# PKU-EPIC/GAPartNet

Measured on AMD Instinct MI355X. Metric: point-clouds/sec (20k pts, train step), higher is better.
Workload: dtype f32

## Files before the change

gapartnet_amd/_C.py:

```python
import ctypes
import os
import subprocess

_HERE = os.path.dirname(os.path.abspath(__file__))
SO_PATH = os.path.join(_HERE, "libgpn_hip.so")
CSRC = os.path.join(_HERE, "csrc")

_lib = None

_SIZE_T_FUNCS = (
    "gpn_voxelize_ws_bytes", "gpn_voxelize_scenes_ws_bytes", "gpn_rulebook_subm3_ws_bytes", "gpn_rulebook_down_ws_bytes",
    "gpn_rulebook_down_lists_ws_bytes", "gpn_rulebook_level_counts_ws_bytes", "gpn_spconv_fwd_ws_bytes", "gpn_spconv_fwd_w_ws_bytes", "gpn_net_ws_bytes", "gpn_linear_bwd_ws_bytes", "gpn_ball_query_grid_ws_bytes", "gpn_point_losses_ws_bytes", "gpn_rulebook_tile_order_ws_bytes", "gpn_bn_ws_bytes", "gpn_spconv_wgrad_ws_bytes", "gpn_ccl_ws_bytes", "gpn_nms_ws_bytes", "gpn_pn2_furthest_point_sampling_ws_bytes", "gpn_pose_fit_ws_bytes", "gpn_proposals_revoxelize_ws_bytes", "gpn_proposals_postprocess_ws_bytes", "gpn_backbone_prepare_arena_bytes", "gpn_scene_prepare_ws_bytes",
    "gpn_view_fps_ws_bytes", "gpn_net_forward_bf16_ws_bytes", "gpn_scene_maps_ws_bytes", "gpn_boxes_draw_ws_bytes",
    "gpn_pointmlp_wgrad_ws_bytes", "gpn_cloud_nearest_ws_bytes", "gpn_proposals_from_masks_ws_bytes",
    "gpn_render_ws_bytes", "gpn_frame_select_ws_bytes", "gpn_ground_mask_resize_ws_bytes", "gpn_ground_knn_ws_bytes",
    "gpn_cloud_grid_sample_ws_bytes",
)


class GpnError(RuntimeError):
    pass


def build(jobs: int = 8) -> str:
# ... 6 lines not shown
    if _lib is None:
        if not os.path.exists(SO_PATH):
            raise GpnError(
                f"{SO_PATH} is missing: the HIP extension has not been built. Run "
                "`python -c 'import __graft_entry__ as g; g.build()'` (needs hipcc). There is no CPU fallback.")
        import torch
        _lib = ctypes.CDLL(SO_PATH)
        _lib.gpn_last_error.restype = ctypes.c_char_p
        _lib.gpn_entry_point_name.restype = ctypes.c_char_p
        for name in _SIZE_T_FUNCS:
            getattr(_lib, name).restype = ctypes.c_size_t
        vp, i64t, i32t, f32t, st = ctypes.c_void_p, ctypes.c_int64, ctypes.c_int, ctypes.c_float, ctypes.c_size_t
        _lib.gpn_spconv_fwd_w.argtypes = [vp, vp, i32t, i32t, i32t, i32t, vp, i64t, vp, vp, st, vp]
        _lib.gpn_spconv_wgrad.argtypes = [vp, vp, vp, vp, vp, i32t, i64t, i32t, i32t, i32t, vp, vp, st, vp]
        _lib.gpn_bn_fwd_train.argtypes = [vp, vp, vp, vp, i64t, i32t, f32t, f32t, i32t, vp, vp, vp, vp, vp, vp, st, vp]
        _lib.gpn_bn_fwd_eval.argtypes = [vp, vp, vp, vp, vp, vp, i64t, i32t, i32t, vp, vp]
        _lib.gpn_bn_bwd.argtypes = [vp, vp, vp, vp, vp, vp, i64t, i32t, i32t, i32t, vp, vp, vp, vp, vp, st, vp]
        _lib.gpn_gather_rows.argtypes = [vp, vp, i64t, i32t, vp, vp]
        _lib.gpn_scatter_rows_csr.argtypes = [vp, vp, vp, i64t, i32t, vp, vp]
        _lib.gpn_spconv_tiles_min_tiles.argtypes = [i64t]
        _lib.gpn_spconv_tiles_min_tiles.restype = i64t
        _lib.gpn_spconv_direct_split.argtypes = [i64t, i64t]
        _lib.gpn_spconv_msplit.argtypes = [i32t, i32t, i32t]
    return _lib


def check(rc: int, what: str = ""):
    if rc != 0:
        msg = lib().gpn_last_error().decode("utf-8", "replace")
        raise GpnError(f"{what or 'gpn call'} failed (code {rc}): {msg}")


def ptr(t):
    if t is None:
        return ctypes.c_void_p(0)
    return ctypes.c_void_p(t.data_ptr())


def i64(v):
    return ctypes.c_int64(int(v))


def i32(v):
    return ctypes.c_int(int(v))


# ... 15 lines not shown
```

gapartnet_amd/csrc/gpn_core.hip:

```cpp
#include <cstdarg>
#include <algorithm>
#include <mutex>
#include <vector>

#include "gpn_common.h"

namespace {
thread_local char g_err[512] = "";

struct ProfRec {
  hipEvent_t a, b;
  int64_t tag;
};
struct ProfLive {
  const int64_t* rows_dev;
  int64_t bound;
  double flops, bytes;
};
struct ProfSlot {
  std::vector<ProfRec> recs;
  std::vector<ProfLive> live;
  double flops = 0, bytes = 0;
  int64_t launches = 0;
};
std::mutex g_prof_mu;
bool g_prof_on = false;
ProfSlot g_prof[GPN_K_COUNT];

const char* kEntryPoints[] = {
    "gpn_voxelize", "gpn_voxelize_ws_bytes", "gpn_rulebook_subm3", "gpn_rulebook_subm3_ws_bytes",
    "gpn_rulebook_down", "gpn_rulebook_down_ws_bytes", "gpn_rulebook_down_lists",
    "gpn_rulebook_down_lists_ws_bytes", "gpn_rulebook_level_counts", "gpn_rulebook_identity", "gpn_rulebook_level_counts_ws_bytes", "gpn_voxelize_ex", "gpn_voxelize_scenes", "gpn_voxelize_scenes_sorted", "gpn_voxelize_scenes_ws_bytes", "gpn_spconv_pack_weights", "gpn_spconv_fwd", "gpn_spconv_fwd_ws_bytes", "gpn_spconv_fwd_route", "gpn_spconv_fwd_ordered", "gpn_rulebook_tile_order_ws_bytes", "gpn_rulebook_tile_order", "gpn_spconv_tiles_min_tiles", "gpn_spconv_direct_split", "gpn_spconv_msplit", "gpn_spconv_fwd_w", "gpn_spconv_fwd_w_ws_bytes", "gpn_spconv_wgrad",
    "gpn_spconv_wgrad_ws_bytes", "gpn_gather_rows", "gpn_scatter_rows_csr", "gpn_bn_ws_bytes", "gpn_bn_fwd_train", "gpn_bn_fwd_eval", "gpn_bn_bwd", "gpn_net_ws_bytes", "gpn_net_bn_fusion", "gpn_net_wgrad_group", "gpn_net_forward", "gpn_linear_supported", "gpn_linear_fwd", "gpn_linear_bwd_ws_bytes", "gpn_linear_bwd", "gpn_net_backward", "gpn_net_forward_pair", "gpn_net_backward_pair", "gpn_point_losses_ws_bytes", "gpn_point_losses_fwd", "gpn_point_losses_fwd_metrics", "gpn_point_losses_bwd", "gpn_score_loss", "gpn_npcs_loss_fwd", "gpn_npcs_loss_bwd", "gpn_ball_query", "gpn_ball_query_grid_ws_bytes", "gpn_ball_query_grid", "gpn_ccl",
    "gpn_ccl_ws_bytes", "gpn_segmented_reduce", "gpn_segmented_maxpool_fwd", "gpn_segmented_maxpool_bwd",
    "gpn_instance_iou", "gpn_nms", "gpn_nms_ws_bytes", "gpn_pn2_ball_query", "gpn_pn2_group_points",
    "gpn_pn2_group_points_grad", "gpn_pn2_gather_points", "gpn_pn2_gather_points_grad",
    "gpn_pn2_furthest_point_sampling", "gpn_pn2_furthest_point_sampling_ws_bytes",
    "gpn_pn2_furthest_point_sampling_ws", "gpn_pn2_three_nn", "gpn_pn2_knn", "gpn_pn2_three_interpolate",
    "gpn_pn2_three_interpolate_grad", "gpn_proposals_max_proposals", "gpn_proposals_build_ws_bytes", "gpn_proposals_build", "gpn_proposals_voxel_mean",
    "gpn_proposals_voxel_mean_bwd", "gpn_proposals_revoxelize_ws_bytes", "gpn_proposals_revoxelize", "gpn_proposals_postprocess_ws_bytes", "gpn_proposals_postprocess", "gpn_proposals_postprocess_lds_proposals", "gpn_backbone_prepare_desc_words", "gpn_backbone_prepare_arena_bytes", "gpn_backbone_prepare", "gpn_scene_prepare_max_instances", "gpn_scene_prepare_ws_bytes", "gpn_scene_prepare", "gpn_pose_fit_ws_bytes", "gpn_pose_fit", "gpn_copy_many", "gpn_adam_blocks", "gpn_adam_step", "gpn_adam_step_gated", "gpn_prof_enable", "gpn_prof_bracket_overhead_us", "gpn_prof_reset", "gpn_prof_get", "gpn_prof_get_launches",
    "gpn_rulebook_subm3_dev", "gpn_rulebook_down_dev_ws_bytes", "gpn_rulebook_down_dev", "gpn_rulebook_down_lists_dev", "gpn_rulebook_identity_dev", "gpn_gather_rows_dev", "gpn_scatter_rows_csr_dev", "gpn_proposals_voxel_mean_dev", "gpn_proposals_targets_dev", "gpn_linear_fwd_dev", "gpn_linear_bwd_dev", "gpn_segmented_maxpool_fwd_dev", "gpn_segmented_maxpool_bwd_dev", "gpn_instance_iou_dev", "gpn_score_loss_dev", "gpn_npcs_loss_fwd_dev", "gpn_npcs_loss_bwd_dev",
    "gpn_view_max_instance_ids", "gpn_view_backproject", "gpn_view_fps_ws_bytes", "gpn_view_fps", "gpn_view_finish",
    "gpn_spconv_pack_weights_bf16", "gpn_spconv_fwd_bf16", "gpn_rows_to_bf16", "gpn_bn_act_bf16", "gpn_net_forward_bf16_ws_bytes",
    "gpn_net_forward_bf16",
    "gpn_scene_maps_ws_bytes", "gpn_scene_maps", "gpn_points_winner", "gpn_points_paint", "gpn_boxes_draw_ws_bytes", "gpn_boxes_draw",
    "gpn_pointmlp_supported", "gpn_pointmlp_fwd", "gpn_pointmlp_wgrad_ws_bytes", "gpn_pointmlp_wgrad",
    "gpn_cloud_pack", "gpn_cloud_finish", "gpn_cloud_nearest_ws_bytes", "gpn_cloud_nearest",
    "gpn_mask_pack", "gpn_proposals_from_masks_ws_bytes", "gpn_proposals_from_masks",
    "gpn_frame_backproject", "gpn_frame_select_ws_bytes", "gpn_frame_select",
    "gpn_cloud_grid_sample_ws_bytes", "gpn_cloud_grid_sample",
    "gpn_joint_sample", "gpn_cpd_rigid", "gpn_joint_from_rigid",
    "gpn_pose_gt_fit", "gpn_box_iou_3d", "gpn_pose_pair_errors",
    "gpn_render_max_links", "gpn_render_ws_bytes", "gpn_render_setup", "gpn_render_raster", "gpn_render_annotate",
    "gpn_render_max_lights", "gpn_render_shade",
    "gpn_ground_mask_resize_ws_bytes", "gpn_ground_mask_resize", "gpn_ground_mask_pool", "gpn_ground_bank_norms",
    "gpn_ground_knn_ws_bytes", "gpn_ground_knn",
// ... 135 lines not shown
```

gapartnet_amd/csrc/net.hip:

```cpp
#include <unistd.h>

#include <cstdlib>

#include <algorithm>
#include <atomic>
#include <condition_variable>
#include <mutex>
#include <string>
#include <thread>
#include <vector>

#include "gpn_common.h"
#include "spconv_pack.h"

namespace {

constexpr int kThreads = 256;

std::atomic<int> g_bn_fusion{1};

struct ConcatPtrs {
  const float4* a;
  const float4* b;
  float4* dst;
};
__global__ __launch_bounds__(kThreads) void concat_kernel(ConcatPtrs pa, ConcatPtrs pb, int64_t rows, int ca4, int cb4,
                                                          const int64_t* __restrict__ rows_dev) {
  rows = gpn::live_rows(rows_dev, rows);
  const ConcatPtrs& p = blockIdx.y ? pb : pa;
  const float4* __restrict__ a = p.a;
  const float4* __restrict__ b = p.b;
  float4* __restrict__ dst = p.dst;
  const int c4 = ca4 + cb4;
  const int64_t total = rows * c4;
  for (int64_t i = (int64_t)blockIdx.x * kThreads + threadIdx.x; i < total; i += (int64_t)gridDim.x * kThreads) {
    const int64_t r = i / c4;
    const int c = (int)(i - r * c4);
    dst[i] = c < ca4 ? a[r * ca4 + c] : b[r * cb4 + (c - ca4)];
  }
}

struct SplitPtrs {
// ... 50 lines not shown
  const PackDesc d = batch.d[blockIdx.y];
  const int64_t total = (int64_t)d.K * d.cin_w * d.cout_w;
  for (int64_t t = (int64_t)blockIdx.x * kThreads + threadIdx.x; t < total; t += (int64_t)gridDim.x * kThreads)
    d.packed[t] = gpn::packed_weight_element(d.W, d.K, d.cin_w, d.cout_w, d.flags, t);
}

inline int grid_for(int64_t total) {
  int64_t g = gpn::cdiv(total, kThreads);
  return (int)(g < 1 ? 1 : (g > 4096 ? 4096 : g));
}

inline size_t slot_bytes(const gpn_net_slot_t& s) { return (size_t)s.rows * s.channels * sizeof(float); }
inline gpn::DevRows dev_rows(const gpn_net_slot_t& s) { return gpn::DevRows{s.rows_dev, s.rows_plan}; }
inline int64_t plan_of(const gpn_net_slot_t& s) { return gpn::plan_rows(s.rows, dev_rows(s)); }

constexpr size_t kWgradBatchBytes = (size_t)96 << 20;

struct Need {
  size_t tmp = 0;
  size_t op = 0;
  size_t wgrad = 0;
  size_t packed = 0;
  size_t stats = 0;
};

Need workspace_need(const gpn_net_op_t* ops, int n_ops, const gpn_net_slot_t* slots, const gpn_net_rulebook_t* rbs,
                    const gpn_net_conv_t* convs) {
  Need n;
  size_t wgrad_sum = 0;
  for (int i = 0; i < n_ops; ++i) {
    const gpn_net_op_t& op = ops[i];
    const gpn_net_slot_t& s0 = slots[op.src0];
    if (op.kind == GPN_NET_CONV) {
      const gpn_net_rulebook_t& rb = rbs[op.rulebook];
      const gpn_net_conv_t& cv = convs[op.param];
      size_t w = gpn_spconv_fwd_ws_bytes(rb.K, rb.n_dst, cv.cin, cv.cout);
      size_t wt = gpn_spconv_fwd_ws_bytes(rb.K, rb.n_src, cv.cout, cv.cin);
      n.op = std::max(n.op, std::max(w, wt));
      const size_t wg = gpn_spconv_wgrad_ws_bytes(rb.K, cv.cin, cv.cout, rb.n_dst);
      n.wgrad = std::max(n.wgrad, wg);
      wgrad_sum += wg;
      n.packed += gpn::align_up((size_t)rb.K * cv.cin * cv.cout * sizeof(float));
      n.tmp = std::max(n.tmp, slot_bytes(s0));
    } else if (op.kind == GPN_NET_BN) {
      n.op = std::max(n.op, gpn_bn_ws_bytes(s0.rows, s0.channels));
      n.stats += gpn::stat_slab_bytes(s0.channels);
      if (op.src1 >= 0) n.tmp = std::max(n.tmp, slot_bytes(slots[op.src1]));
    }
  }
  n.tmp = gpn::align_up(n.tmp);
  n.op = gpn::align_up(n.op);
  n.wgrad = gpn::align_up(std::max(n.wgrad, std::min(wgrad_sum, kWgradBatchBytes)));
  return n;
}

int pack_program(const gpn_net_op_t* ops, int n_ops, const gpn_net_rulebook_t* rbs, const gpn_net_conv_t* convs,
                 bool transposed, char* area, std::vector<const float*>& packed_of, hipStream_t stream) {
  packed_of.assign(n_ops, nullptr);
  PackBatch batch;
  int fill = 0;
  int64_t max_total = 0;
  size_t off = 0;
  auto flush = [&]() -> int {
    if (fill == 0) return GPN_OK;
    int gx = (int)std::min<int64_t>(gpn::cdiv(max_total, kThreads), 256);
    hipLaunchKernelGGL(pack_many_kernel, dim3(gx, fill), dim3(kThreads), 0, stream, batch);
    hipError_t e = hipGetLastError();
    if (e != hipSuccess) {
      gpn::set_error("gpn_net: weight packing launch failed: %s", hipGetErrorString(e));
      return GPN_ERR_HIP;
    }
    fill = 0;
    max_total = 0;
    return GPN_OK;
  };
// ... 79 lines not shown
  return GPN_OK;
}

}

extern "C" int gpn_net_bn_fusion(int on) {
  return on < 0 ? g_bn_fusion.load(std::memory_order_relaxed) : g_bn_fusion.exchange(on ? 1 : 0, std::memory_order_relaxed);
}

namespace {
std::atomic<int>& wgrad_group_setting();
}
extern "C" int gpn_net_wgrad_group(int layers) {
  std::atomic<int>& g = wgrad_group_setting();
  if (layers < 1) return g.load(std::memory_order_relaxed);
  return g.exchange(layers > gpn::kWgradSets ? gpn::kWgradSets : layers, std::memory_order_relaxed);
}

extern "C" size_t gpn_net_ws_bytes(const gpn_net_op_t* ops, int n_ops, const gpn_net_slot_t* slots, int n_slots,
                                   const gpn_net_rulebook_t* rulebooks, const gpn_net_conv_t* convs) {
  (void)n_slots;
  if (!ops || !slots) return 0;
  const Need n = workspace_need(ops, n_ops, slots, rulebooks, convs);
  return n.tmp + n.op + n.wgrad + n.packed + n.stats;
}

namespace {

struct NetSet {
  gpn_net_slot_t* slots;
  const gpn_net_conv_t* convs;
  const gpn_net_bn_t* bns;
};

int net_forward_impl(const char* who, const gpn_net_op_t* ops, int n_ops, const NetSet* nets, int n_nets, int n_slots,
                     const gpn_net_rulebook_t* rbs, int n_rbs, int n_convs, int n_bns, int mode, void* ws, size_t ws_bytes,
                     hipStream_t stream) {
  const int training = mode == 1 ? 1 : 0;
  const bool inference = mode == GPN_NET_INFERENCE;
  if (mode != 0 && mode != 1 && mode != GPN_NET_INFERENCE) {
    gpn::set_error("%s: training must be 0, 1 or GPN_NET_INFERENCE", who);
    return GPN_ERR_ARG;
  }
  int rc = GPN_OK;
  for (int t = 0; t < n_nets; ++t) {
    rc = check_program(who, ops, n_ops, nets[t].slots, n_slots, rbs, n_rbs, nets[t].convs, n_convs, nets[t].bns, n_bns);
    if (rc) return rc;
// ... 181 lines not shown
                          (hipStream_t)stream_);
}

namespace {

std::atomic<int> g_wgrad_group{4};
std::atomic<int>& wgrad_group_setting() { return g_wgrad_group; }

constexpr int64_t g_wgrad_group_rows = 16384;

struct WgradJob {
  const float* in;
  const float* dout;
  const int32_t *pair_src, *pair_dst, *tile_off;
  int K;
  int64_t n_dst;
  gpn::DevRows rows;
  int cin, cout;
  float* dW;
  hipEvent_t after;
  const float* in2;
  const float* dout2;
  float* dW2;
};

class WgradWorker {
 public:
  void begin(int dev, hipStream_t side, void* ws, size_t ws_bytes, size_t max_jobs) {
    ensure_thread();
    jobs_.resize(max_jobs);
    dev_ = dev, side_ = side, ws_ = ws, ws_bytes_ = ws_bytes;
    published_.store(0, std::memory_order_relaxed);
    closed_.store(false, std::memory_order_relaxed);
    finished_.store(false, std::memory_order_relaxed);
    rc_ = GPN_OK;
    {
      std::lock_guard<std::mutex> lk(mu_);
      active_ = true;
    }
    cv_.notify_one();
  }
  void push(const WgradJob& j) {
    const size_t i = published_.load(std::memory_order_relaxed);
    jobs_[i] = j;
    published_.store(i + 1, std::memory_order_release);
  }
  int finish(std::string& err) {
    closed_.store(true, std::memory_order_release);
    while (!finished_.load(std::memory_order_acquire)) std::this_thread::yield();
    err = err_;
    return rc_;
  }

 private:
  void ensure_thread() {
    const pid_t pid = getpid();
    if (started_ && pid_ == pid) return;
    started_ = true;
    pid_ = pid;
    std::thread([this] { run(); }).detach();
  }
  void run() {
    for (;;) {
      {
        std::unique_lock<std::mutex> lk(mu_);
        cv_.wait(lk, [this] { return active_; });
        active_ = false;
      }
      (void)hipSetDevice(dev_);
      size_t done = 0;
      gpn::WgradReduceJob pending[gpn::kWgradReduceJobs];
      int n_pending = 0;
      size_t used = 0;
      const size_t room = std::min(ws_bytes_, kWgradBatchBytes);
      auto fail = [this](int rc) {
        if (rc_ == GPN_OK) {
          rc_ = rc;
          err_ = gpn_last_error();
        }
      };
      auto flush = [&] {
        if (n_pending && rc_ == GPN_OK) {
          const int rc = gpn::wgrad_reduce_many(pending, n_pending, side_);
          if (rc != GPN_OK) fail(rc);
        }
        n_pending = 0;
        used = 0;
      };
      WgradJob group[gpn::kWgradSets];
      int n_group = 0, group_sets = 0;
      auto same_shape = [](const WgradJob& a, const WgradJob& b) {
        return a.K == b.K && a.n_dst == b.n_dst && a.cin == b.cin && a.cout == b.cout && a.rows.dev == b.rows.dev;
      };
      auto launch_group = [&]() -> int {
        if (!n_group) return GPN_OK;
        const WgradJob& j0 = group[0];
        const int n = n_group, n_sets = group_sets;
        n_group = 0, group_sets = 0;
        if (hipStreamWaitEvent(side_, group[n - 1].after, 0) != hipSuccess) {
          gpn::set_error("gpn_net_backward: hipStreamWaitEvent failed on the weight-gradient stream");
          return GPN_ERR_HIP;
        }
        const size_t elems = (size_t)j0.K * j0.cin * j0.cout;
        if (j0.n_dst == 0) {
          for (int g = 0; g < n; ++g) {
            GPN_CHECK_HIP(hipMemsetAsync(group[g].dW, 0, sizeof(float) * elems, side_));
            if (group[g].dW2) GPN_CHECK_HIP(hipMemsetAsync(group[g].dW2, 0, sizeof(float) * elems, side_));
          }
          return GPN_OK;
        }
        const int S = gpn::wgrad_slices(j0.K, j0.cin, j0.cout, gpn::plan_rows(j0.n_dst, j0.rows));
        const size_t bytes = gpn::align_up((size_t)S * elems * sizeof(float));
        if (used + n_sets * bytes > room || n_pending + n_sets > gpn::kWgradReduceJobs) flush();
        if (n_sets * bytes > ws_bytes_ || !ws_) {
          gpn::set_error("gpn_net_backward: weight-gradient workspace too small");
          return GPN_ERR_WS;
        }
        gpn::WgradSets sets;
        float* dW_of[gpn::kWgradSets];
        for (int g = 0; g < n; ++g) {
          const WgradJob& j = group[g];
          float* partial = reinterpret_cast<float*>(static_cast<char*>(ws_) + used + sets.n * bytes);
          dW_of[sets.n] = j.dW;
          sets.s[sets.n++] = gpn::WgradSet{j.in, j.dout, j.pair_src, j.pair_dst, j.tile_off, partial};
          if (j.dW2) {
            partial = reinterpret_cast<float*>(static_cast<char*>(ws_) + used + sets.n * bytes);
            dW_of[sets.n] = j.dW2;
            sets.s[sets.n++] = gpn::WgradSet{j.in2, j.dout2, j.pair_src, j.pair_dst, j.tile_off, partial};
          }
        }
        const int rc = gpn::wgrad_contract(sets, j0.K, j0.n_dst, j0.cin, j0.cout, S, side_, j0.rows.dev);
        if (rc != GPN_OK) return rc;
        for (int q = 0; q < sets.n; ++q)
          pending[n_pending++] = gpn::wgrad_reduce_job(sets.s[q].partial, S, j0.K, j0.cin, j0.cout, GPN_LAYOUT_OKI, dW_of[q]);
        used += sets.n * bytes;
        return GPN_OK;
      };
      auto issue = [&](const WgradJob& j) -> int {
        const int n_sets = j.dW2 ? 2 : 1;
        const int limit = gpn::plan_rows(j.n_dst, j.rows) < g_wgrad_group_rows ? g_wgrad_group.load(std::memory_order_relaxed) : 1;
        if (n_group && (!same_shape(group[0], j) || group_sets + n_sets > limit)) {
          const int rc = launch_group();
          if (rc != GPN_OK) return rc;
        }
        group[n_group++] = j;
        group_sets += n_sets;
        if (group_sets >= limit) return launch_group();
        return GPN_OK;
      };
      for (;;) {
        const size_t avail = published_.load(std::memory_order_acquire);
        if (done < avail) {
          const WgradJob& j = jobs_[done++];
          if (rc_ != GPN_OK) continue;
          const int rc = issue(j);
          if (rc != GPN_OK) fail(rc);
        } else if (closed_.load(std::memory_order_acquire) && done == published_.load(std::memory_order_acquire)) {
          break;
        } else {
          std::this_thread::yield();
        }
      }
      if (rc_ == GPN_OK) {
        const int rc = launch_group();
        if (rc != GPN_OK) fail(rc);
      }
      flush();
      finished_.store(true, std::memory_order_release);
    }
  }

  std::mutex mu_;
  std::condition_variable cv_;
  bool active_ = false, started_ = false;
  pid_t pid_ = 0;
  std::vector<WgradJob> jobs_;
  std::atomic<size_t> published_{0};
  std::atomic<bool> closed_{false}, finished_{false};
  int dev_ = 0;
  hipStream_t side_ = nullptr;
  void* ws_ = nullptr;
  size_t ws_bytes_ = 0;
  int rc_ = GPN_OK;
  std::string err_;
};

struct DeviceWorker {
  std::mutex pass_mu;
  WgradWorker worker;
};

DeviceWorker& device_worker(int dev) {
  static std::mutex mu;
  static DeviceWorker* per_device[gpn::kMaxDevices] = {};
  std::lock_guard<std::mutex> lk(mu);
  if (!per_device[dev]) per_device[dev] = new DeviceWorker();
  return *per_device[dev];
}

struct GradTarget {
  float* ptr;
  bool staged;
};

inline GradTarget grad_target(gpn_net_slot_t& s, float* tmp) {
// ... 9 lines not shown
    if (e != hipSuccess) {
      gpn::set_error("gpn_net_backward: accumulate launch failed: %s", hipGetErrorString(e));
      return GPN_ERR_HIP;
    }
  }
  s.grad_state = 1;
  return GPN_OK;
}

}

namespace {

int net_backward_impl(const char* who, const gpn_net_op_t* ops, int n_ops, const NetSet* nets, int n_nets, int n_slots,
                      const gpn_net_rulebook_t* rbs, int n_rbs, int n_convs, int n_bns, int training, int need_input_grad,
                      void* ws, size_t ws_bytes, hipStream_t stream) {
  int rc = GPN_OK;
  for (int t = 0; t < n_nets; ++t) {
    rc = check_program(who, ops, n_ops, nets[t].slots, n_slots, rbs, n_rbs, nets[t].convs, n_convs, nets[t].bns, n_bns);
    if (rc) return rc;
  }
  const Need need = workspace_need(ops, n_ops, nets[0].slots, rbs, nets[0].convs);
  const size_t per_net = need.tmp + need.packed + need.stats;
  const size_t total_need = n_nets * per_net + need.op + n_nets * need.wgrad;
  if (!ws || ws_bytes < total_need) {
    gpn::set_error("%s: workspace too small (%zu needed, %zu given)", who, total_need, ws_bytes);
    return GPN_ERR_WS;
  }
  char* base = static_cast<char*>(ws);
  float* tmp[2] = {reinterpret_cast<float*>(base), reinterpret_cast<float*>(base + per_net)};
  void* op_ws = base + n_nets * per_net;
  const size_t op_ws_bytes = need.op;
  void* wgrad_ws = base + n_nets * per_net + need.op;
  const size_t wgrad_ws_bytes = ws_bytes - (n_nets * per_net + need.op);
  std::vector<const float*> packed_of[2];
  for (int t = 0; t < n_nets; ++t) {
    rc = pack_program(ops, n_ops, rbs, nets[t].convs, true, base + t * per_net + need.tmp, packed_of[t], stream);
    if (rc) return rc;
  }
  std::vector<unsigned long long*> bn_slab[2];
  for (int t = 0; t < n_nets; ++t) bn_slab[t].assign(n_ops, nullptr);
  std::vector<int> fused_by(n_ops, -1);
  std::vector<char> sums_done(n_ops, 0);
  if (g_bn_fusion.load(std::memory_order_relaxed)) {
    std::vector<int> first_reader(n_slots, -1), producer(n_slots, -1);
    for (int i = n_ops - 1; i >= 0; --i) {
      first_reader[ops[i].src0] = i;
      if (ops[i].src1 >= 0) first_reader[ops[i].src1] = i;
      producer[ops[i].dst] = i;
    }
    size_t off = 0;
    for (int i = 0; i < n_ops; ++i) {
      if (ops[i].kind != GPN_NET_CONV) continue;
      const int j = producer[ops[i].src0];
      if (j < 0 || ops[j].kind != GPN_NET_BN || first_reader[ops[i].src0] != i) continue;
      if (ops[i].src0 == 0 && !need_input_grad) continue;
      const gpn_net_rulebook_t& rb = rbs[ops[i].rulebook];
// ... 4 lines not shown
        continue;
      for (int t = 0; t < n_nets; ++t)
        bn_slab[t][j] = reinterpret_cast<unsigned long long*>(base + t * per_net + need.tmp + need.packed + off);
      off += gpn::stat_slab_bytes(cv.cin);
      fused_by[i] = j;
    }
    if (off)
      for (int t = 0; t < n_nets; ++t) GPN_CHECK_HIP(hipMemsetAsync(base + t * per_net + need.tmp + need.packed, 0, off, stream));
  }
  SideStream* side = side_stream();
  if (!side) {
    gpn::set_error("%s: could not create the weight-gradient stream", who);
    return GPN_ERR_HIP;
  }
  GPN_CHECK_HIP(hipEventRecord(side->join, side->stream));
  GPN_CHECK_HIP(hipStreamWaitEvent(stream, side->join, 0));
  bool forked = false;
  int device = 0;
  GPN_CHECK_HIP(hipGetDevice(&device));
  GPN_CHECK_ARG(device >= 0 && device < gpn::kMaxDevices);
  DeviceWorker& dw = device_worker(device);
  std::lock_guard<std::mutex> pass_lock(dw.pass_mu);
  WgradWorker& worker = dw.worker;
  worker.begin(device, side->stream, wgrad_ws, wgrad_ws_bytes, (size_t)n_ops * n_nets);
  struct PassGuard {
    WgradWorker& w;
    bool closed = false;
    ~PassGuard() {
      if (!closed) {
        std::string ignored;
        (void)w.finish(ignored);
      }
    }
  } guard{worker};
  const bool pair = n_nets == 2;
  for (int i = n_ops - 1; i >= 0; --i) {
    const gpn_net_op_t& op = ops[i];
    gpn_net_slot_t &s0 = nets[0].slots[op.src0], &d = nets[0].slots[op.dst];
    if (!d.grad_state) continue;
    for (int t = 0; t < n_nets; ++t) {
      const gpn_net_slot_t &ts0 = nets[t].slots[op.src0], &td = nets[t].slots[op.dst];
      if (!td.grad || !ts0.data || !td.data || td.grad_state != d.grad_state) {
        gpn::set_error("%s: op %d: null pointer (or the two networks' gradient states differ)", who, i);
        return GPN_ERR_ARG;
      }
    }
    if (op.kind == GPN_NET_CONV) {
      const gpn_net_rulebook_t& rb = rbs[op.rulebook];
      const gpn_net_conv_t& cv = nets[0].convs[op.param];
      bool any_dw = false;
      for (int t = 0; t < n_nets; ++t) any_dw = any_dw || nets[t].convs[op.param].dW;
      if (any_dw) {
        if (!rb.pair_src || !rb.pair_dst || !rb.tile_off) {
          gpn::set_error("%s: op %d: rulebook has no pair lists for wgrad", who, i);
          return GPN_ERR_ARG;
        }
        hipEvent_t ev = side->fork[side->next];
        side->next = (side->next + 1) % kForkEvents;
        GPN_CHECK_HIP(hipEventRecord(ev, stream));
        if (pair && nets[0].convs[op.param].dW && nets[1].convs[op.param].dW) {
          worker.push(WgradJob{nets[0].slots[op.src0].data, nets[0].slots[op.dst].grad, rb.pair_src, rb.pair_dst, rb.tile_off,
                               rb.K, rb.n_dst, dev_rows(d), cv.cin, cv.cout, nets[0].convs[op.param].dW, ev, nets[1].slots[op.src0].data,
                               nets[1].slots[op.dst].grad, nets[1].convs[op.param].dW});
        } else {
          for (int t = 0; t < n_nets; ++t)
            if (nets[t].convs[op.param].dW)
              worker.push(WgradJob{nets[t].slots[op.src0].data, nets[t].slots[op.dst].grad, rb.pair_src, rb.pair_dst, rb.tile_off,
                                   rb.K, rb.n_dst, dev_rows(d), cv.cin, cv.cout, nets[t].convs[op.param].dW, ev, nullptr, nullptr, nullptr});
        }
        forked = true;
      }
      if (op.src0 != 0 || need_input_grad) {
        for (int t = 0; t < n_nets; ++t)
          if (!nets[t].slots[op.src0].grad || !rb.nbr_t) {
            gpn::set_error("%s: op %d: null gradient buffer / transposed table", who, i);
            return GPN_ERR_ARG;
          }
        gpn::ConvStats st;
        if (pair) {
          st.twin.in = nets[1].slots[op.dst].grad;
          st.twin.packed = packed_of[1][i];
          st.twin.out = nets[1].slots[op.src0].grad;
        }
        if (fused_by[i] >= 0) {
          const gpn_net_op_t& bo = ops[fused_by[i]];
          const gpn_net_bn_t& bn = nets[0].bns[bo.param];
          st.slab = bn_slab[0][fused_by[i]];
          st.slot_mask = gpn::stat_slot_count(plan_of(s0)) - 1;
          st.x = nets[0].slots[bo.src0].data;
          st.y = s0.data;
          st.mean = training ? bn.save_mean : bn.running_mean;
          st.invstd = bn.save_invstd;
// ... 59 lines not shown
        nets[t].slots[op.src0].grad_state = 1;
        if (pp[t].dres) {
          rc = commit(nets[t].slots[op.src1], tr[t], stream);
          if (rc) return rc;
        }
      }
    } else {
      gpn_net_slot_t& s1 = nets[0].slots[op.src1];
      for (int t = 0; t < n_nets; ++t)
        if (!nets[t].slots[op.src0].grad || !nets[t].slots[op.src1].grad) {
          gpn::set_error("%s: op %d: null gradient buffer", who, i);
          return GPN_ERR_ARG;
        }
      SplitPtrs sa{(const float4*)d.grad, (float4*)s0.grad, (float4*)s1.grad}, sb = sa;
      if (pair)
        sb = SplitPtrs{(const float4*)nets[1].slots[op.dst].grad, (float4*)nets[1].slots[op.src0].grad,
                       (float4*)nets[1].slots[op.src1].grad};
      hipLaunchKernelGGL(split_kernel, dim3(grid_for(plan_of(d) * (d.channels / 4)), n_nets), dim3(kThreads), 0, stream, sa, sb, d.rows,
                         s0.channels / 4, s1.channels / 4, s0.grad_state, s1.grad_state, d.rows_dev);
      GPN_CHECK_LAUNCH();
      for (int t = 0; t < n_nets; ++t) nets[t].slots[op.src0].grad_state = nets[t].slots[op.src1].grad_state = 1;
    }
  }
  std::string worker_err;
  guard.closed = true;
  rc = worker.finish(worker_err);
  if (rc) {
    gpn::set_error("%s", worker_err.c_str());
    return rc;
  }
  if (forked) {
    GPN_CHECK_HIP(hipEventRecord(side->join, side->stream));
    GPN_CHECK_HIP(hipStreamWaitEvent(stream, side->join, 0));
  }
  return GPN_OK;
}

}

extern "C" int gpn_net_backward(const gpn_net_op_t* ops, int n_ops, gpn_net_slot_t* slots, int n_slots,
                                const gpn_net_rulebook_t* rbs, int n_rbs, const gpn_net_conv_t* convs, int n_convs,
                                const gpn_net_bn_t* bns, int n_bns, int training, int need_input_grad, void* ws,
                                size_t ws_bytes, gpn_stream_t stream_) {
  const NetSet one{slots, convs, bns};
  return net_backward_impl(__func__, ops, n_ops, &one, 1, n_slots, rbs, n_rbs, n_convs, n_bns, training, need_input_grad, ws,
                           ws_bytes, (hipStream_t)stream_);
}

extern "C" int gpn_net_backward_pair(const gpn_net_op_t* ops, int n_ops, gpn_net_slot_t* slots_a, gpn_net_slot_t* slots_b,
                                     int n_slots, const gpn_net_rulebook_t* rbs, int n_rbs, const gpn_net_conv_t* convs_a,
                                     const gpn_net_conv_t* convs_b, int n_convs, const gpn_net_bn_t* bns_a,
                                     const gpn_net_bn_t* bns_b, int n_bns, int training, int need_input_grad, void* ws,
// ... 191 lines not shown
```

include/gpn.h:

```cpp
#ifndef GPN_H
#define GPN_H

#include <stddef.h>
#include <stdint.h>

#ifdef __cplusplus
extern "C" {
#endif

typedef void* gpn_stream_t;

#define GPN_OK 0
#define GPN_ERR_ARG 1
#define GPN_ERR_WS 2
#define GPN_ERR_HIP 3

const char* gpn_last_error(void);
int gpn_version(void);
int gpn_num_entry_points(void);
const char* gpn_entry_point_name(int i);

int gpn_linear_supported(int cin, int cout);
int gpn_linear_fwd(const float* x, const float* W, const float* b, int64_t N, int cin, int cout, float* y, gpn_stream_t stream);
size_t gpn_linear_bwd_ws_bytes(int64_t N, int cin, int cout);
// ... 161 lines not shown
  float* dbias;
  float eps;
  float momentum;
  int32_t C;
  int32_t reserved;
} gpn_net_bn_t;
#define GPN_NET_CONV 0
#define GPN_NET_BN 1
#define GPN_NET_CONCAT 2
#define GPN_NET_RELU 1
#define GPN_NET_INFERENCE 2
typedef struct gpn_net_op {
  int32_t kind;
  int32_t src0;
  int32_t src1;
  int32_t dst;
  int32_t rulebook;
  int32_t param;
  int32_t flags;
  int32_t reserved;
} gpn_net_op_t;
int gpn_net_bn_fusion(int on);
int gpn_net_wgrad_group(int layers);
size_t gpn_net_ws_bytes(const gpn_net_op_t* ops, int n_ops, const gpn_net_slot_t* slots, int n_slots,
                        const gpn_net_rulebook_t* rulebooks, const gpn_net_conv_t* convs);
int gpn_net_forward(const gpn_net_op_t* ops, int n_ops, gpn_net_slot_t* slots, int n_slots,
                    const gpn_net_rulebook_t* rulebooks, int n_rulebooks, const gpn_net_conv_t* convs, int n_convs,
                    const gpn_net_bn_t* bns, int n_bns, int training, void* ws, size_t ws_bytes, gpn_stream_t stream);
int gpn_net_backward(const gpn_net_op_t* ops, int n_ops, gpn_net_slot_t* slots, int n_slots,
                     const gpn_net_rulebook_t* rulebooks, int n_rulebooks, const gpn_net_conv_t* convs, int n_convs,
                     const gpn_net_bn_t* bns, int n_bns, int training, int need_input_grad, void* ws, size_t ws_bytes,
                     gpn_stream_t stream);
int gpn_net_forward_pair(const gpn_net_op_t* ops, int n_ops, gpn_net_slot_t* slots_a, gpn_net_slot_t* slots_b, int n_slots,
                         const gpn_net_rulebook_t* rulebooks, int n_rulebooks, const gpn_net_conv_t* convs_a,
                         const gpn_net_conv_t* convs_b, int n_convs, const gpn_net_bn_t* bns_a, const gpn_net_bn_t* bns_b,
                         int n_bns, int training, void* ws, size_t ws_bytes, gpn_stream_t stream);
int gpn_net_backward_pair(const gpn_net_op_t* ops, int n_ops, gpn_net_slot_t* slots_a, gpn_net_slot_t* slots_b, int n_slots,
                          const gpn_net_rulebook_t* rulebooks, int n_rulebooks, const gpn_net_conv_t* convs_a,
                          const gpn_net_conv_t* convs_b, int n_convs, const gpn_net_bn_t* bns_a, const gpn_net_bn_t* bns_b,
                          int n_bns, int training, int need_input_grad, void* ws, size_t ws_bytes, gpn_stream_t stream);

typedef struct gpn_conv_epilogue_bf16 {
  const float* mean;
  const float* var;
  const float* weight;
  const float* bias;
// ... 362 lines not shown
```

Measured before the change: 1048.

## Add deferred weight-gradient scheduling and move grouping decisions to the main thread

Adds an opt-in mode that holds weight-gradient jobs for the first high-resolution conv layers of the backward pass in a separate workspace. They are released as a batch once the pass descends to coarser levels, so they can overlap with later backward work. Grouping decisions move from the worker thread to the issuing thread, which records one fork event per closed group instead of one per conv. The default path also changes, since fewer events are recorded. A stats entry point reports deferred and eager counts, events and groups; the cost is extra workspace and more complex control flow.

```diff
diff --git a/gapartnet_amd/_C.py b/gapartnet_amd/_C.py
--- a/gapartnet_amd/_C.py
+++ b/gapartnet_amd/_C.py
@@ -52,6 +52,8 @@
         _lib.gpn_spconv_tiles_min_tiles.restype = i64t
         _lib.gpn_spconv_direct_split.argtypes = [i64t, i64t]
         _lib.gpn_spconv_msplit.argtypes = [i32t, i32t, i32t]
+        _lib.gpn_net_wgrad_defer.argtypes = [i32t, i64t]
+        _lib.gpn_net_backward_stats.argtypes = [ctypes.POINTER(i64t * 4)]
     return _lib
 
 
diff --git a/gapartnet_amd/csrc/gpn_core.hip b/gapartnet_amd/csrc/gpn_core.hip
--- a/gapartnet_amd/csrc/gpn_core.hip
+++ b/gapartnet_amd/csrc/gpn_core.hip
@@ -31,7 +31,7 @@
     "gpn_voxelize", "gpn_voxelize_ws_bytes", "gpn_rulebook_subm3", "gpn_rulebook_subm3_ws_bytes",
     "gpn_rulebook_down", "gpn_rulebook_down_ws_bytes", "gpn_rulebook_down_lists",
     "gpn_rulebook_down_lists_ws_bytes", "gpn_rulebook_level_counts", "gpn_rulebook_identity", "gpn_rulebook_level_counts_ws_bytes", "gpn_voxelize_ex", "gpn_voxelize_scenes", "gpn_voxelize_scenes_sorted", "gpn_voxelize_scenes_ws_bytes", "gpn_spconv_pack_weights", "gpn_spconv_fwd", "gpn_spconv_fwd_ws_bytes", "gpn_spconv_fwd_route", "gpn_spconv_fwd_ordered", "gpn_rulebook_tile_order_ws_bytes", "gpn_rulebook_tile_order", "gpn_spconv_tiles_min_tiles", "gpn_spconv_direct_split", "gpn_spconv_msplit", "gpn_spconv_fwd_w", "gpn_spconv_fwd_w_ws_bytes", "gpn_spconv_wgrad",
-    "gpn_spconv_wgrad_ws_bytes", "gpn_gather_rows", "gpn_scatter_rows_csr", "gpn_bn_ws_bytes", "gpn_bn_fwd_train", "gpn_bn_fwd_eval", "gpn_bn_bwd", "gpn_net_ws_bytes", "gpn_net_bn_fusion", "gpn_net_wgrad_group", "gpn_net_forward", "gpn_linear_supported", "gpn_linear_fwd", "gpn_linear_bwd_ws_bytes", "gpn_linear_bwd", "gpn_net_backward", "gpn_net_forward_pair", "gpn_net_backward_pair", "gpn_point_losses_ws_bytes", "gpn_point_losses_fwd", "gpn_point_losses_fwd_metrics", "gpn_point_losses_bwd", "gpn_score_loss", "gpn_npcs_loss_fwd", "gpn_npcs_loss_bwd", "gpn_ball_query", "gpn_ball_query_grid_ws_bytes", "gpn_ball_query_grid", "gpn_ccl",
+    "gpn_spconv_wgrad_ws_bytes", "gpn_gather_rows", "gpn_scatter_rows_csr", "gpn_bn_ws_bytes", "gpn_bn_fwd_train", "gpn_bn_fwd_eval", "gpn_bn_bwd", "gpn_net_ws_bytes", "gpn_net_bn_fusion", "gpn_net_wgrad_group", "gpn_net_wgrad_defer", "gpn_net_backward_stats", "gpn_net_forward", "gpn_linear_supported", "gpn_linear_fwd", "gpn_linear_bwd_ws_bytes", "gpn_linear_bwd", "gpn_net_backward", "gpn_net_forward_pair", "gpn_net_backward_pair", "gpn_point_losses_ws_bytes", "gpn_point_losses_fwd", "gpn_point_losses_fwd_metrics", "gpn_point_losses_bwd", "gpn_score_loss", "gpn_npcs_loss_fwd", "gpn_npcs_loss_bwd", "gpn_ball_query", "gpn_ball_query_grid_ws_bytes", "gpn_ball_query_grid", "gpn_ccl",
     "gpn_ccl_ws_bytes", "gpn_segmented_reduce", "gpn_segmented_maxpool_fwd", "gpn_segmented_maxpool_bwd",
     "gpn_instance_iou", "gpn_nms", "gpn_nms_ws_bytes", "gpn_pn2_ball_query", "gpn_pn2_group_points",
     "gpn_pn2_group_points_grad", "gpn_pn2_gather_points", "gpn_pn2_gather_points_grad",
diff --git a/gapartnet_amd/csrc/net.hip b/gapartnet_amd/csrc/net.hip
--- a/gapartnet_amd/csrc/net.hip
+++ b/gapartnet_amd/csrc/net.hip
@@ -18,6 +18,9 @@
 constexpr int kThreads = 256;
 
 std::atomic<int> g_bn_fusion{1};
+
+std::atomic<int> g_wgrad_defer{0};
+std::atomic<int64_t> g_wgrad_defer_rows{16384};
 
 struct ConcatPtrs {
   const float4* a;
@@ -114,7 +117,10 @@
   size_t wgrad = 0;
   size_t packed = 0;
   size_t stats = 0;
+  size_t held = 0;
 };
+
+constexpr int kWgradHeldSets = gpn::kWgradReduceJobs;
 
 Need workspace_need(const gpn_net_op_t* ops, int n_ops, const gpn_net_slot_t* slots, const gpn_net_rulebook_t* rbs,
                     const gpn_net_conv_t* convs) {
@@ -143,6 +149,19 @@
   n.tmp = gpn::align_up(n.tmp);
   n.op = gpn::align_up(n.op);
   n.wgrad = gpn::align_up(std::max(n.wgrad, std::min(wgrad_sum, kWgradBatchBytes)));
+  if (g_wgrad_defer.load(std::memory_order_relaxed)) {
+    const int64_t min_rows = g_wgrad_defer_rows.load(std::memory_order_relaxed);
+    int layers = 0;
+    for (int i = n_ops - 1; i >= 0 && layers < kWgradHeldSets; --i) {
+      if (ops[i].kind != GPN_NET_CONV) continue;
+      if (plan_of(slots[ops[i].dst]) < min_rows) break;
+      const gpn_net_rulebook_t& rb = rbs[ops[i].rulebook];
+      const gpn_net_conv_t& cv = convs[ops[i].param];
+      n.held += gpn_spconv_wgrad_ws_bytes(rb.K, cv.cin, cv.cout, rb.n_dst);
+      ++layers;
+    }
+    n.held = gpn::align_up(std::min(n.held, kWgradBatchBytes));
+  }
   return n;
 }
 
@@ -268,7 +287,35 @@
   (void)n_slots;
   if (!ops || !slots) return 0;
   const Need n = workspace_need(ops, n_ops, slots, rulebooks, convs);
-  return n.tmp + n.op + n.wgrad + n.packed + n.stats;
+  return n.tmp + n.op + n.wgrad + n.packed + n.stats + n.held;
+}
+
+extern "C" int gpn_net_wgrad_defer(int mode, int64_t min_rows) {
+  if (mode < 0) return g_wgrad_defer.load(std::memory_order_relaxed);
+  if (min_rows >= 1) g_wgrad_defer_rows.store(min_rows, std::memory_order_relaxed);
+  return g_wgrad_defer.exchange(mode ? 1 : 0, std::memory_order_relaxed);
+}
+
+namespace {
+struct BackwardStats {
+  std::mutex mu;
+  int64_t v[gpn::kMaxDevices][4] = {};
+};
+BackwardStats& backward_stats() {
+  static BackwardStats s;
+  return s;
+}
+}
+
+extern "C" int gpn_net_backward_stats(int64_t out[4]) {
+  GPN_CHECK_ARG(out);
+  int dev = 0;
+  GPN_CHECK_HIP(hipGetDevice(&dev));
+  GPN_CHECK_ARG(dev >= 0 && dev < gpn::kMaxDevices);
+  BackwardStats& s = backward_stats();
+  std::lock_guard<std::mutex> lk(s.mu);
+  std::copy(s.v[dev], s.v[dev] + 4, out);
+  return GPN_OK;
 }
 
 namespace {
@@ -496,14 +543,41 @@
   const float* in2;
   const float* dout2;
   float* dW2;
+  int kind = 0;
+  int sets() const { return dW2 ? 2 : 1; }
+};
+
+enum { kWgradJob = 0, kWgradFence, kWgradHeld, kWgradRelease, kWgradFlush };
+
+inline WgradJob wgrad_marker(int kind, hipEvent_t after) {
+  WgradJob m{};
+  m.kind = kind, m.after = after;
+  return m;
+}
+
+struct WgradGrouping {
+  int layers;
+  WgradJob first{};
+  int n = 0, sets = 0;
+  static bool same_shape(const WgradJob& a, const WgradJob& b) {
+    return a.K == b.K && a.n_dst == b.n_dst && a.cin == b.cin && a.cout == b.cout && a.rows.dev == b.rows.dev;
+  }
+  int limit(const WgradJob& j) const { return gpn::plan_rows(j.n_dst, j.rows) < g_wgrad_group_rows ? layers : 1; }
+  bool closes_before(const WgradJob& j) const { return n && (!same_shape(first, j) || sets + j.sets() > limit(j)); }
+  bool add(const WgradJob& j) {
+    if (!n) first = j;
+    ++n, sets += j.sets();
+    return sets >= limit(j);
+  }
+  void close() { n = 0, sets = 0; }
 };
 
 class WgradWorker {
  public:
-  void begin(int dev, hipStream_t side, void* ws, size_t ws_bytes, size_t max_jobs) {
+  void begin(int dev, hipStream_t side, void* ws, size_t ws_bytes, void* held_ws, size_t held_bytes, int layers, size_t max_entries) {
     ensure_thread();
-    jobs_.resize(max_jobs);
-    dev_ = dev, side_ = side, ws_ = ws, ws_bytes_ = ws_bytes;
+    jobs_.resize(max_entries);
+    dev_ = dev, side_ = side, ws_ = ws, ws_bytes_ = ws_bytes, held_ws_ = held_ws, held_bytes_ = held_bytes, layers_ = layers;
     published_.store(0, std::memory_order_relaxed);
     closed_.store(false, std::memory_order_relaxed);
     finished_.store(false, std::memory_order_relaxed);
@@ -525,8 +599,16 @@
     err = err_;
     return rc_;
   }
+  int64_t groups() const { return groups_; }
 
  private:
+  struct Lane {
+    char* ws;
+    size_t bytes, room;
+    size_t used = 0;
+    gpn::WgradReduceJob pending[gpn::kWgradReduceJobs];
+    int n_pending = 0;
+  };
   void ensure_thread() {
     const pid_t pid = getpid();
     if (started_ && pid_ == pid) return;
@@ -543,38 +625,35 @@
       }
       (void)hipSetDevice(dev_);
       size_t done = 0;
-      gpn::WgradReduceJob pending[gpn::kWgradReduceJobs];
-      int n_pending = 0;
-      size_t used = 0;
-      const size_t room = std::min(ws_bytes_, kWgradBatchBytes);
+      Lane eager{static_cast<char*>(ws_), ws_bytes_, std::min(ws_bytes_, kWgradBatchBytes)};
+      Lane held{static_cast<char*>(held_ws_), held_bytes_, held_bytes_};
+      held_jobs_.clear();
+      groups_ = 0;
       auto fail = [this](int rc) {
         if (rc_ == GPN_OK) {
           rc_ = rc;
           err_ = gpn_last_error();
         }
       };
-      auto flush = [&] {
-        if (n_pending && rc_ == GPN_OK) {
-          const int rc = gpn::wgrad_reduce_many(pending, n_pending, side_);
+      auto flush = [&](Lane& l) {
+        if (l.n_pending && rc_ == GPN_OK) {
+          const int rc = gpn::wgrad_reduce_many(l.pending, l.n_pending, side_);
           if (rc != GPN_OK) fail(rc);
         }
-        n_pending = 0;
-        used = 0;
+        l.n_pending = 0;
+        l.used = 0;
       };
-      WgradJob group[gpn::kWgradSets];
-      int n_group = 0, group_sets = 0;
-      auto same_shape = [](const WgradJob& a, const WgradJob& b) {
-        return a.K == b.K && a.n_dst == b.n_dst && a.cin == b.cin && a.cout == b.cout && a.rows.dev == b.rows.dev;
-      };
-      auto launch_group = [&]() -> int {
-        if (!n_group) return GPN_OK;
-        const WgradJob& j0 = group[0];
-        const int n = n_group, n_sets = group_sets;
-        n_group = 0, group_sets = 0;
-        if (hipStreamWaitEvent(side_, group[n - 1].after, 0) != hipSuccess) {
+      auto wait_for = [&](hipEvent_t after) -> int {
+        if (hipStreamWaitEvent(side_, after, 0) != hipSuccess) {
           gpn::set_error("gpn_net_backward: hipStreamWaitEvent failed on the weight-gradient stream");
           return GPN_ERR_HIP;
         }
+        return GPN_OK;
+      };
+      auto launch_group = [&](Lane& l, const WgradJob* group, int n, int n_sets) -> int {
+        if (!n) return GPN_OK;
+        ++groups_;
+        const WgradJob& j0 = group[0];
         const size_t elems = (size_t)j0.K * j0.cin * j0.cout;
         if (j0.n_dst == 0) {
           for (int g = 0; g < n; ++g) {
@@ -585,8 +664,8 @@
         }
         const int S = gpn::wgrad_slices(j0.K, j0.cin, j0.cout, gpn::plan_rows(j0.n_dst, j0.rows));
         const size_t bytes = gpn::align_up((size_t)S * elems * sizeof(float));
-        if (used + n_sets * bytes > room || n_pending + n_sets > gpn::kWgradReduceJobs) flush();
-        if (n_sets * bytes > ws_bytes_ || !ws_) {
+        if (l.used + n_sets * bytes > l.room || l.n_pending + n_sets > gpn::kWgradReduceJobs) flush(l);
+        if (n_sets * bytes > l.bytes || !l.ws) {
           gpn::set_error("gpn_net_backward: weight-gradient workspace too small");
           return GPN_ERR_WS;
         }
@@ -594,11 +673,11 @@
         float* dW_of[gpn::kWgradSets];
         for (int g = 0; g < n; ++g) {
           const WgradJob& j = group[g];
-          float* partial = reinterpret_cast<float*>(static_cast<char*>(ws_) + used + sets.n * bytes);
+          float* partial = reinterpret_cast<float*>(l.ws + l.used + sets.n * bytes);
           dW_of[sets.n] = j.dW;
           sets.s[sets.n++] = gpn::WgradSet{j.in, j.dout, j.pair_src, j.pair_dst, j.tile_off, partial};
           if (j.dW2) {
-            partial = reinterpret_cast<float*>(static_cast<char*>(ws_) + used + sets.n * bytes);
+            partial = reinterpret_cast<float*>(l.ws + l.used + sets.n * bytes);
             dW_of[sets.n] = j.dW2;
             sets.s[sets.n++] = gpn::WgradSet{j.in2, j.dout2, j.pair_src, j.pair_dst, j.tile_off, partial};
           }
@@ -606,28 +685,66 @@
         const int rc = gpn::wgrad_contract(sets, j0.K, j0.n_dst, j0.cin, j0.cout, S, side_, j0.rows.dev);
         if (rc != GPN_OK) return rc;
         for (int q = 0; q < sets.n; ++q)
-          pending[n_pending++] = gpn::wgrad_reduce_job(sets.s[q].partial, S, j0.K, j0.cin, j0.cout, GPN_LAYOUT_OKI, dW_of[q]);
-        used += sets.n * bytes;
+          l.pending[l.n_pending++] = gpn::wgrad_reduce_job(sets.s[q].partial, S, j0.K, j0.cin, j0.cout, GPN_LAYOUT_OKI, dW_of[q]);
+        l.used += sets.n * bytes;
         return GPN_OK;
       };
-      auto issue = [&](const WgradJob& j) -> int {
-        const int n_sets = j.dW2 ? 2 : 1;
-        const int limit = gpn::plan_rows(j.n_dst, j.rows) < g_wgrad_group_rows ? g_wgrad_group.load(std::memory_order_relaxed) : 1;
-        if (n_group && (!same_shape(group[0], j) || group_sets + n_sets > limit)) {
-          const int rc = launch_group();
-          if (rc != GPN_OK) return rc;
-        }
-        group[n_group++] = j;
-        group_sets += n_sets;
-        if (group_sets >= limit) return launch_group();
-        return GPN_OK;
+      WgradJob group[gpn::kWgradSets];
+      WgradGrouping open{layers_};
+      auto release = [&](hipEvent_t after) -> int {
+        int rc = after ? wait_for(after) : GPN_OK;
+        WgradJob hgroup[gpn::kWgradSets];
+        WgradGrouping g{layers_};
+        for (size_t i = 0; i < held_jobs_.size() && rc == GPN_OK; ++i) {
+          const WgradJob& j = held_jobs_[i];
+          if (g.closes_before(j)) {
+            rc = launch_group(held, hgroup, g.n, g.sets);
+            g.close();
+            if (rc != GPN_OK) break;
+          }
+          hgroup[g.n] = j;
+          if (g.add(j)) {
+            rc = launch_group(held, hgroup, g.n, g.sets);
+            g.close();
+          }
+        }
+        if (rc == GPN_OK) rc = launch_group(held, hgroup, g.n, g.sets);
+        held_jobs_.clear();
+        if (rc == GPN_OK) flush(held);
+        return rc;
+      };
+      auto handle = [&](const WgradJob& e) -> int {
+        switch (e.kind) {
+          case kWgradJob:
+            if (open.closes_before(e) || open.n == gpn::kWgradSets) {
+              gpn::set_error("gpn_net_backward: a weight-gradient group was not closed where the grouping rule closes it");
+              return GPN_ERR_ARG;
+            }
+            group[open.n] = e;
+            open.add(e);
+            return GPN_OK;
+          case kWgradFence: {
+            int rc = wait_for(e.after);
+            if (rc == GPN_OK) rc = launch_group(eager, group, open.n, open.sets);
+            open.close();
+            return rc;
+          }
+          case kWgradHeld:
+            held_jobs_.push_back(e);
+            return GPN_OK;
+          case kWgradRelease:
+            return release(e.after);
+          default:
+            flush(eager);
+            return GPN_OK;
+        }
       };
       for (;;) {
         const size_t avail = published_.load(std::memory_order_acquire);
         if (done < avail) {
-          const WgradJob& j = jobs_[done++];
+          const WgradJob& e = jobs_[done++];
           if (rc_ != GPN_OK) continue;
-          const int rc = issue(j);
+          const int rc = handle(e);
           if (rc != GPN_OK) fail(rc);
         } else if (closed_.load(std::memory_order_acquire) && done == published_.load(std::memory_order_acquire)) {
           break;
@@ -635,11 +752,7 @@
           std::this_thread::yield();
         }
       }
-      if (rc_ == GPN_OK) {
-        const int rc = launch_group();
-        if (rc != GPN_OK) fail(rc);
-      }
-      flush();
+      flush(eager);
       finished_.store(true, std::memory_order_release);
     }
   }
@@ -655,6 +768,11 @@
   hipStream_t side_ = nullptr;
   void* ws_ = nullptr;
   size_t ws_bytes_ = 0;
+  void* held_ws_ = nullptr;
+  size_t held_bytes_ = 0;
+  int layers_ = 1;
+  std::vector<WgradJob> held_jobs_;
+  int64_t groups_ = 0;
   int rc_ = GPN_OK;
   std::string err_;
 };
@@ -710,7 +828,8 @@
   }
   const Need need = workspace_need(ops, n_ops, nets[0].slots, rbs, nets[0].convs);
   const size_t per_net = need.tmp + need.packed + need.stats;
-  const size_t total_need = n_nets * per_net + need.op + n_nets * need.wgrad;
+  const size_t held_bytes = n_nets * need.held;
+  const size_t total_need = n_nets * per_net + need.op + n_nets * need.wgrad + held_bytes;
   if (!ws || ws_bytes < total_need) {
     gpn::set_error("%s: workspace too small (%zu needed, %zu given)", who, total_need, ws_bytes);
     return GPN_ERR_WS;
@@ -719,8 +838,9 @@
   float* tmp[2] = {reinterpret_cast<float*>(base), reinterpret_cast<float*>(base + per_net)};
   void* op_ws = base + n_nets * per_net;
   const size_t op_ws_bytes = need.op;
-  void* wgrad_ws = base + n_nets * per_net + need.op;
-  const size_t wgrad_ws_bytes = ws_bytes - (n_nets * per_net + need.op);
+  void* held_ws = base + n_nets * per_net + need.op;
+  void* wgrad_ws = base + n_nets * per_net + need.op + held_bytes;
+  const size_t wgrad_ws_bytes = ws_bytes - (n_nets * per_net + need.op + held_bytes);
   std::vector<const float*> packed_of[2];
   for (int t = 0; t < n_nets; ++t) {
     rc = pack_program(ops, n_ops, rbs, nets[t].convs, true, base + t * per_net + need.tmp, packed_of[t], stream);
@@ -771,7 +891,8 @@
   DeviceWorker& dw = device_worker(device);
   std::lock_guard<std::mutex> pass_lock(dw.pass_mu);
   WgradWorker& worker = dw.worker;
-  worker.begin(device, side->stream, wgrad_ws, wgrad_ws_bytes, (size_t)n_ops * n_nets);
+  WgradGrouping open{g_wgrad_group.load(std::memory_order_relaxed)};
+  worker.begin(device, side->stream, wgrad_ws, wgrad_ws_bytes, held_ws, held_bytes, open.layers, (size_t)n_ops * (2 * n_nets + 1) + 4);
   struct PassGuard {
     WgradWorker& w;
     bool closed = false;
@@ -783,6 +904,58 @@
     }
   } guard{worker};
   const bool pair = n_nets == 2;
+  const int64_t defer_rows = g_wgrad_defer_rows.load(std::memory_order_relaxed);
+  bool descended = false;
+  int64_t level_rows = -1;
+  int held_sets = 0;
+  size_t held_used = 0;
+  int64_t n_deferred = 0, n_eager = 0, n_events = 0;
+  auto fork_event = [&](hipEvent_t* ev) -> int {
+    *ev = side->fork[side->next];
+    side->next = (side->next + 1) % kForkEvents;
+    GPN_CHECK_HIP(hipEventRecord(*ev, stream));
+    ++n_events;
+    return GPN_OK;
+  };
+  auto close_group = [&]() -> int {
+    if (!open.n) return GPN_OK;
+    hipEvent_t ev;
+    const int rc = fork_event(&ev);
+    if (rc) return rc;
+    worker.push(wgrad_marker(kWgradFence, ev));
+    open.close();
+    return GPN_OK;
+  };
+  auto release = [&]() -> int {
+    if (!held_sets) return GPN_OK;
+    hipEvent_t ev = nullptr;
+    const int rc = open.n ? close_group() : fork_event(&ev);
+    if (rc) return rc;
+    worker.push(wgrad_marker(kWgradRelease, ev));
+    held_sets = 0;
+    return GPN_OK;
+  };
+  auto publish = [&](WgradJob j) -> int {
+    if (held_bytes && !descended) {
+      const size_t elems = (size_t)j.K * j.cin * j.cout;
+      const int S = j.n_dst ? gpn::wgrad_slices(j.K, j.cin, j.cout, gpn::plan_rows(j.n_dst, j.rows)) : 0;
+      const size_t bytes = j.sets() * gpn::align_up((size_t)S * elems * sizeof(float));
+      if (held_sets + j.sets() <= kWgradHeldSets && held_used + bytes <= held_bytes) {
+        j.kind = kWgradHeld;
+        worker.push(j);
+        held_sets += j.sets(), held_used += bytes;
+        ++n_deferred;
+        return GPN_OK;
+      }
+    }
+    if (open.closes_before(j)) {
+      const int rc = close_group();
+      if (rc) return rc;
+    }
+    worker.push(j);
+    ++n_eager;
+    return open.add(j) ? close_group() : GPN_OK;
+  };
   for (int i = n_ops - 1; i >= 0; --i) {
     const gpn_net_op_t& op = ops[i];
     gpn_net_slot_t &s0 = nets[0].slots[op.src0], &d = nets[0].slots[op.dst];
@@ -797,6 +970,17 @@
     if (op.kind == GPN_NET_CONV) {
       const gpn_net_rulebook_t& rb = rbs[op.rulebook];
       const gpn_net_conv_t& cv = nets[0].convs[op.param];
+      const int64_t dst_rows = plan_of(d);
+      if (!descended && dst_rows < defer_rows) {
+        descended = true;
+        rc = release();
+        if (rc) return rc;
+      } else if (descended && dst_rows >= defer_rows && dst_rows != level_rows && forked) {
+        rc = close_group();
+        if (rc) return rc;
+        worker.push(wgrad_marker(kWgradFlush, nullptr));
+      }
+      level_rows = dst_rows;
       bool any_dw = false;
       for (int t = 0; t < n_nets; ++t) any_dw = any_dw || nets[t].convs[op.param].dW;
       if (any_dw) {
@@ -804,19 +988,18 @@
           gpn::set_error("%s: op %d: rulebook has no pair lists for wgrad", who, i);
           return GPN_ERR_ARG;
         }
-        hipEvent_t ev = side->fork[side->next];
-        side->next = (side->next + 1) % kForkEvents;
-        GPN_CHECK_HIP(hipEventRecord(ev, stream));
         if (pair && nets[0].convs[op.param].dW && nets[1].convs[op.param].dW) {
-          worker.push(WgradJob{nets[0].slots[op.src0].data, nets[0].slots[op.dst].grad, rb.pair_src, rb.pair_dst, rb.tile_off,
-                               rb.K, rb.n_dst, dev_rows(d), cv.cin, cv.cout, nets[0].convs[op.param].dW, ev, nets[1].slots[op.src0].data,
-                               nets[1].slots[op.dst].grad, nets[1].convs[op.param].dW});
+          rc = publish(WgradJob{nets[0].slots[op.src0].data, nets[0].slots[op.dst].grad, rb.pair_src, rb.pair_dst, rb.tile_off,
+                                rb.K, rb.n_dst, dev_rows(d), cv.cin, cv.cout, nets[0].convs[op.param].dW, nullptr,
+                                nets[1].slots[op.src0].data, nets[1].slots[op.dst].grad, nets[1].convs[op.param].dW});
         } else {
-          for (int t = 0; t < n_nets; ++t)
+          for (int t = 0; t < n_nets && rc == GPN_OK; ++t)
             if (nets[t].convs[op.param].dW)
-              worker.push(WgradJob{nets[t].slots[op.src0].data, nets[t].slots[op.dst].grad, rb.pair_src, rb.pair_dst, rb.tile_off,
-                                   rb.K, rb.n_dst, dev_rows(d), cv.cin, cv.cout, nets[t].convs[op.param].dW, ev, nullptr, nullptr, nullptr});
-        }
+              rc = publish(WgradJob{nets[t].slots[op.src0].data, nets[t].slots[op.dst].grad, rb.pair_src, rb.pair_dst, rb.tile_off,
+                                    rb.K, rb.n_dst, dev_rows(d), cv.cin, cv.cout, nets[t].convs[op.param].dW, nullptr, nullptr, nullptr,
+                                    nullptr});
+        }
+        if (rc) return rc;
         forked = true;
       }
       if (op.src0 != 0 || need_input_grad) {
@@ -922,12 +1105,21 @@
       for (int t = 0; t < n_nets; ++t) nets[t].slots[op.src0].grad_state = nets[t].slots[op.src1].grad_state = 1;
     }
   }
+  rc = release();
+  if (rc == GPN_OK) rc = close_group();
+  if (rc) return rc;
   std::string worker_err;
   guard.closed = true;
   rc = worker.finish(worker_err);
   if (rc) {
     gpn::set_error("%s", worker_err.c_str());
     return rc;
+  }
+  {
+    BackwardStats& s = backward_stats();
+    std::lock_guard<std::mutex> lk(s.mu);
+    const int64_t v[4] = {n_deferred, n_eager, n_events, worker.groups()};
+    std::copy(v, v + 4, s.v[device]);
   }
   if (forked) {
     GPN_CHECK_HIP(hipEventRecord(side->join, side->stream));
diff --git a/include/gpn.h b/include/gpn.h
--- a/include/gpn.h
+++ b/include/gpn.h
@@ -207,6 +207,8 @@
 } gpn_net_op_t;
 int gpn_net_bn_fusion(int on);
 int gpn_net_wgrad_group(int layers);
+int gpn_net_wgrad_defer(int mode, int64_t min_rows);
+int gpn_net_backward_stats(int64_t out[4]);
 size_t gpn_net_ws_bytes(const gpn_net_op_t* ops, int n_ops, const gpn_net_slot_t* slots, int n_slots,
                         const gpn_net_rulebook_t* rulebooks, const gpn_net_conv_t* convs);
 int gpn_net_forward(const gpn_net_op_t* ops, int n_ops, gpn_net_slot_t* slots, int n_slots,
```

New measurement: 1058, median of 6. About the same (+1.0%).
